# mirage/decompress

Hardware: AMD Instinct MI355X
Metric: MiB/s inflate over N zlib streams (uncompressed bytes / wall second) (higher is better)
Workload: dtype u8; 1 GPU; C2: 4096 x 256 KiB zlib streams per GPU, dynamic Huffman (libz level 6; even streams = slices of the reference's test/corpus, odd = order-2 Markov ASCII text, 64 symbols, seed 0xC2 + i, SURVEY 8(d)), Zl.Inf.Ns semantics, one stream per pair of wavefronts (decoder + copier); streams_per_gpu=4096, stream_bytes=262144, unique_streams=4096

## Files before the change

### decompress_amd/csrc/inflate_wave.hip

```cpp
#ifndef MD_RMAX
#define MD_RMAX 576
#endif
#ifndef MD_STAGE
#define MD_STAGE 5248
#endif
#ifndef MD_PAIR_OCC
#define MD_PAIR_OCC 5
#endif
#include "inflate_wave_core.hpp"

namespace md {
namespace wv {

#ifdef MD_DEBUG_KNOWN_BOUNDS
constexpr uint32_t KB_ROUNDS = 512;
__device__ uint4 *g_kb_buf;
__device__ int g_kb_mode;
#endif
struct Sink {
  lds_u8 *stage;
  uint8_t *g;
  uint32_t cap;
  uint32_t pos;
  uint32_t lane;
  uint32_t a, b;
  bool want_adler;
  __device__ __forceinline__ uint32_t sbase() const { return pos & ~15u; }

  __device__ __forceinline__ void flush(uint32_t total) {
    const uint32_t rb = sbase();
    const uint32_t endp = pos + total;
    const uint32_t full0 = (pos + 15) & ~15u, full1 = endp & ~15u;
    uint32_t s1 = 0, s2 = 0;
    for (uint32_t ps = full0; ps < full1; ps += 1024) {
      const uint32_t cpos = ps + lane * 16;
      if (cpos < full1) {
        const lds_u32 *sp = reinterpret_cast<const lds_u32 *>(stage + (cpos - rb));
        const uint32_t w0 = sp[0], w1 = sp[1], w2 = sp[2], w3 = sp[3];
        const uint4 v = make_uint4(w0, w1, w2, w3);
        __builtin_memcpy(g + cpos, &v, 16);
        if (want_adler) {
          uint32_t t1 = __builtin_amdgcn_udot4(w0, 0x01010101u, 0u, false);
          t1 = __builtin_amdgcn_udot4(w1, 0x01010101u, t1, false);
          t1 = __builtin_amdgcn_udot4(w2, 0x01010101u, t1, false);
          t1 = __builtin_amdgcn_udot4(w3, 0x01010101u, t1, false);
          uint32_t tk = __builtin_amdgcn_udot4(w0, 0x03020100u, 0u, false);
          tk = __builtin_amdgcn_udot4(w1, 0x07060504u, tk, false);
          tk = __builtin_amdgcn_udot4(w2, 0x0b0a0908u, tk, false);
          tk = __builtin_amdgcn_udot4(w3, 0x0f0e0d0cu, tk, false);
          s1 += t1;
          s2 += (endp - cpos) * t1 - tk;
        }
      }
    }
    {
      const uint32_t head1 = full0 < endp ? full0 : endp;
      const uint32_t tail0 = full1 > head1 ? full1 : head1;
      const uint32_t x = lane < 16 ? pos + lane : tail0 + (lane - 16);
      if (lane < 16 ? x < head1 : (lane < 32 && x < endp)) {
        const uint32_t d = stage[x - rb];
        g[x] = (uint8_t)d;
        s1 += d;
        s2 += (endp - x) * d;
      }
    }
    if (want_adler) {
      s1 = wave_sum(s1);
      s2 = wave_sum(s2 % 65521u);
      b = (b + total * a + s2) % 65521u;
      a = (a + s1) % 65521u;
    }
    pos = endp;
  }
};

constexpr int FR = RMAX / kWave;
struct FarRow {
  uint32_t qs, n, src;
  bool near, has;
  uint32_t ml;
};
__device__ __forceinline__ FarRow far_row(const lds_u32 *mrec, const lds_u16 *mpos, uint32_t r, uint32_t nrec, uint32_t rb, uint32_t R0) {
  FarRow f;
  f.has = r < nrec;
  const uint32_t tk = mrec[f.has ? r : 0u];
  f.qs = mpos[f.has ? r : 0u];
  const uint32_t d = (tk & 0x7fff) + 1;
  f.ml = ((tk >> 16) & 0xff) + 3;
  const uint32_t s = rb + f.qs - d;
  f.near = f.has && (tk & kNearBit);
  const uint32_t head = s < R0 ? R0 - s : 0u;
  f.n = !f.has ? 0u : f.near ? head : f.ml;
  f.src = f.n ? s : 0u;
  return f;
}
template <class PF>
__device__ __forceinline__ void copy_far(const lds_u32 *mrec, const lds_u16 *mpos, lds_u16 *list, const Sink &sk,
                                         uint32_t lane, uint32_t nrec, uint32_t *nnear_out, PF &pf) {
  lds_u8 *stage = sk.stage;
  const uint32_t R0 = sk.pos, rb = sk.sbase();
  const uint8_t *g = sk.g;
  uint32_t nnear = 0;
  uint64_t v0[FR], v1[FR];
  uint32_t pk[FR];
  uint32_t nlong = 0;
  bool spill = false;
#pragma unroll
  for (int u = 0; u < FR; u++) {
    const FarRow f = far_row(mrec, mpos, u * kWave + lane, nrec, rb, R0);
    v0[u] = out_ld64(g + f.src);
    v1[u] = out_ld64(g + f.src + 8);
    pk[u] = f.qs | (f.n << 16);
    const uint64_t nb = __ballot(f.near);
    if (f.near) list[nnear + lane_rank(nb)] = (uint16_t)(u * kWave + lane);
    nnear += (uint32_t)__builtin_popcountll(nb);
    const uint64_t lb = __ballot(f.n > 16);
    const uint32_t lc = (uint32_t)__builtin_popcountll(lb);
    if (nnear + nlong + lc > RMAX) {
      spill = true;
      nlong = 0;
    }
    if (lb && !spill) {
      if (f.n > 16) list[RMAX - 1 - (nlong + lane_rank(lb))] = (uint16_t)(u * kWave + lane);
      nlong += lc;
    }
  }
  pf.tick_lds(P_FAR_REC);
#pragma unroll
  for (int u = 0; u < FR; u++) {
    if ((uint32_t)u * kWave < nrec) {
      const uint32_t qs = pk[u] & 0xffffu, n = pk[u] >> 16;
      if constexpr (PF::on) {
        if (u == 0) {
          asm volatile("" ::"v"(v0[u]), "v"(v1[u]));
          pf.tick_all(P_FAR_LOAD);
        }
      }
      if (n) {
        lds_u8 *dd = stage + qs;
        lds_put(dd, v0[u], n < 8 ? n : 8);
        if (n > 8) lds_put(dd + 8, v1[u], n < 16 ? n - 8 : 8);
      }
    }
  }
  pf.tick_lds(P_FAR);
  for (uint32_t c0 = 0; c0 < nlong; c0 += kWave) {
    const bool has = c0 + lane < nlong;
    const uint32_t r = has ? list[RMAX - 1 - (c0 + lane)] : 0u;
    const FarRow f = far_row(mrec, mpos, r, nrec, rb, R0);
    const uint32_t n = has ? f.n : 0u;
    const uint64_t w0 = out_ld64(g + (n ? f.src + 16 : 0u)), w1 = out_ld64(g + (n ? f.src + 24 : 0u));
    if (n) {
      lds_u8 *dd = stage + f.qs + 16;
      lds_put(dd, w0, n < 24 ? n - 16 : 8);
      if (n > 24) lds_put(dd + 8, w1, n < 32 ? n - 24 : 8);
    }
    for (uint64_t lm = __ballot(n > 32); lm;) {
      uint32_t ln[4], lsrc[4], lqs[4];
      uint64_t d[4];
#pragma unroll
      for (int k = 0; k < 4; k++) {
        const bool any = lm != 0;
        const uint32_t l = any ? (uint32_t)__builtin_ctzll(lm) : 0u;
        lm &= lm - 1;
        ln[k] = any ? rdlane(n, l) : 0u;
        lsrc[k] = rdlane(f.src, l);
        lqs[k] = rdlane(f.qs, l);
      }
      const uint32_t j = 32 + lane * 8;
#pragma unroll
      for (int k = 0; k < 4; k++) d[k] = out_ld64(g + (j < ln[k] ? lsrc[k] + j : 0u));
#pragma unroll
      for (int k = 0; k < 4; k++)
        if (j < ln[k]) lds_put(stage + lqs[k] + j, d[k], ln[k] - j < 8 ? ln[k] - j : 8);
    }
  }
  if (spill) {
    pf.count(C_FAR_SPILL);
    for (uint32_t c0 = 0; c0 < nrec; c0 += kWave) {
      const FarRow f = far_row(mrec, mpos, c0 + lane, nrec, rb, R0);
      for (uint64_t lm = __ballot(f.n > 16); lm; lm &= lm - 1) {
        const uint32_t l = (uint32_t)__builtin_ctzll(lm);
        const uint32_t ln = rdlane(f.n, l), lsrc = rdlane(f.src, l), lqs = rdlane(f.qs, l);
        const uint32_t j = 16 + lane * 8;
        if (j < ln) lds_put(stage + lqs + j, out_ld64(g + lsrc + j), ln - j < 8 ? ln - j : 8);
      }
    }
  }
  pf.tick_all(P_FAR);
  *nnear_out = nnear;
}
template <class PF>
__device__ __noinline__ void copy_far_guarded(const lds_u32 *mrec, const lds_u16 *mpos, lds_u16 *list,
                                              lds_u8 *stage, const uint8_t *g, uint32_t R0, uint32_t rb, uint32_t cap,
                                              uint32_t lane, uint32_t nrec, uint32_t *nnear_out) {
  uint32_t nnear = 0;
  for (uint32_t c0 = 0; c0 < nrec; c0 += kWave) {
    const uint32_t r = c0 + lane;
    const bool has = r < nrec;
    const uint32_t tk = mrec[has ? r : 0u], qs = mpos[has ? r : 0u];
    const uint32_t d = (tk & 0x7fff) + 1, ml = ((tk >> 16) & 0xff) + 3;
    const uint32_t s = rb + qs - d;
    const bool near = has && (tk & kNearBit);
    uint32_t n = has ? ml : 0u;
    const uint64_t nb = __ballot(near);
    if (near) {
      list[nnear + lane_rank(nb)] = (uint16_t)r;
      n = s < R0 ? R0 - s : 0u;
    }
    nnear += (uint32_t)__builtin_popcountll(nb);
    for (uint32_t j = 0; j < n; j += 8) lds_put(stage + qs + j, out_ld_guard(g, s + j, n - j, cap), n - j < 8 ? n - j : 8);
  }
  *nnear_out = nnear;
}

__device__ __forceinline__ void wave_copy(lds_u8 *stage, uint32_t dd, uint32_t ss, uint32_t n, uint32_t d, uint32_t lane) {
  if (d >= n) {
    const uint32_t j = lane * 8;
    if (j < n) lds_put(stage + dd + j, lds_ld64(stage + ss + j), n - j < 8 ? n - j : 8);
  } else if (d < 8) {
    uint64_t v = lds_ld64(stage + ss);
    const uint32_t sh = 8 * d;
    v &= (1ull << sh) - 1;
    v |= v << sh;
    if (2 * sh < 64) v |= v << (2 * sh);
    if (4 * sh < 64) v |= v << (4 * sh);
    const uint32_t adv = (0x76586880u >> (4 * d)) & 15;
    const uint32_t j = lane * adv;
    if (j < n) lds_put(stage + dd + j, v, n - j < adv ? n - j : adv);
  } else {
    const float inv = 1.0f / (float)d;
    for (uint32_t j = lane * 4; j < n; j += 4 * kWave) {
      uint32_t r = j - (uint32_t)((float)j * inv) * d;
      r = (int32_t)r < 0 ? r + d : r;
      r = r >= d ? r - d : r;
      uint32_t w = 0;
#pragma unroll
      for (uint32_t k = 0; k < 4; k++) {
        const uint32_t x = r + k >= d ? r + k - d : r + k;
        w |= (uint32_t)stage[ss + x] << (8 * k);
      }
      lds_put(stage + dd + j, w, n - j < 4 ? n - j : 4);
    }
  }
}

template <class PF>
__device__ __forceinline__ void copy_near_all(const lds_u32 *mrec, const lds_u16 *mpos, const lds_u16 *list,
                                              const Sink &sk, uint32_t lane, uint32_t count, bool *stuck, PF &pf) {
  lds_u8 *stage = sk.stage;
  const uint32_t head = sk.pos - sk.sbase();
  for (uint32_t c0 = 0; c0 < count; c0 += kWave) {
    bool todo = c0 + lane < count;
    const uint32_t e = todo ? list[c0 + lane] : 0u;
    const uint32_t tk = mrec[e], qs = mpos[e];
    const uint32_t d = (tk & 0x7fff) + 1, ml = ((tk >> 16) & 0xff) + 3;
    const int32_t s0 = (int32_t)qs - (int32_t)d;
    const uint32_t skip = s0 < (int32_t)head ? head - (uint32_t)s0 : 0u;
    const uint32_t sa = (uint32_t)(s0 + (int32_t)skip), sb = d < ml ? qs : (uint32_t)s0 + ml;
    const uint32_t n = ml - skip;
    const bool fast = d >= n && n <= 32;
    const uint32_t qb = todo ? qs + skip : 0xffffffffu, qe = todo ? qs + ml : 0xffffffffu;
    uint32_t jlo = 0, jhi = 0;
#pragma unroll
    for (uint32_t st = 32; st > 0; st >>= 1) {
      const uint32_t ve = __shfl(qe, jlo + st - 1), vb = __shfl(qb, jhi + st - 1);
      jlo = ve <= sa ? jlo + st : jlo;
      jhi = vb < sb ? jhi + st : jhi;
    }
    jhi = jhi < lane ? jhi : lane;
    uint64_t need = 0;
    if (sa < sb && jlo < jhi) need = ((jhi >= 64 ? 0ull : (1ull << jhi)) - 1ull) & ~((1ull << jlo) - 1ull);
    uint64_t done = 0;
    pf.tick_lds(P_NEAR_LOAD);
    for (uint32_t guard = 0; __ballot(todo) != 0; guard++) {
      if (guard > kWave) {
        *stuck = true;
        return;
      }
      pf.count(C_NEAR_IT);
      const bool ready = todo && (need & ~done) == 0;
      if constexpr (PF::on) {
        if (__ballot(ready && !fast)) pf.count(C_LONG_NEAR);
      }
      pf.tick_lds(P_NEAR);
      if (ready && fast) {
        lds_u8 *dd = stage + qs + skip;
        const lds_u8 *ss = stage + sa;
        const uint64_t v0 = lds_ld64(ss), v1 = lds_ld64(ss + 8), v2 = lds_ld64(ss + 16), v3 = lds_ld64(ss + 24);
        lds_put(dd, v0, n < 8 ? n : 8);
        if (n > 8) lds_put(dd + 8, v1, n < 16 ? n - 8 : 8);
        if (n > 16) {
          lds_put(dd + 16, v2, n < 24 ? n - 16 : 8);
          if (n > 24) lds_put(dd + 24, v3, n - 24);
        }
      }
      pf.tick_lds(P_NEAR_FAST);
      for (uint64_t lm = __ballot(ready && !fast); lm; lm &= lm - 1) {
        const uint32_t l = (uint32_t)__builtin_ctzll(lm);
        wave_copy(stage, rdlane(qs + skip, l), rdlane(sa, l), rdlane(n, l), rdlane(d, l), lane);
      }
      pf.tick_lds(P_NEAR_SLOW);
      done |= __ballot(ready);
      todo = todo && !ready;
      pf.tick_lds(P_NEAR_UPD);
    }
  }
  pf.tick(P_NEAR);
}

template <class PF>
__device__ __forceinline__ void copy_round(lds_smem *sm, Sink &sk, uint32_t lane, uint32_t total, uint32_t nrec, bool *stuck, PF &pf) {
  const lds_u32 *mrec = (const lds_u32 *)sm->mrec;
  const lds_u16 *mpos = (const lds_u16 *)sm->mpos;
  lds_u16 *list = (lds_u16 *)sm->list;
  const uint32_t R0 = sk.pos, rb = sk.sbase();
  uint32_t nnear = 0;
#ifdef MD_DEBUG_KNOWN_BOUNDS
  {
    const int kbm = __builtin_amdgcn_readfirstlane(g_kb_mode);
    if (kbm & 8) {
      sk.pos += total;
      return;
    }
    if (kbm & 4) {
      sk.flush(total);
      return;
    }
  }
#endif
  __builtin_amdgcn_fence(__ATOMIC_RELEASE, "workgroup");
  if (R0 + 40 > sk.cap) {
    copy_far_guarded<PF>(mrec, mpos, list, sk.stage, sk.g, R0, rb, sk.cap, lane, nrec, &nnear);
    pf.tick(P_FAR);
  } else {
    copy_far(mrec, mpos, list, sk, lane, nrec, &nnear, pf);
  }
  copy_near_all(mrec, mpos, list, sk, lane, nnear, stuck, pf);
  sk.flush(total);
  pf.tick(P_ADLER);
}

__device__ __forceinline__ uint32_t mail_ld(const MD_LDS uint32_t *p) {
  return __hip_atomic_load(p, __ATOMIC_RELAXED, __HIP_MEMORY_SCOPE_WORKGROUP);
}
__device__ __forceinline__ void mail_st(MD_LDS uint32_t *p, uint32_t v) {
  __hip_atomic_store(p, v, __ATOMIC_RELAXED, __HIP_MEMORY_SCOPE_WORKGROUP);
}
__device__ __forceinline__ bool mail_wait_idle(lds_smem *sm, uint32_t sent) {
  while (uni(mail_ld(&sm->mail.copied)) != sent) __builtin_amdgcn_s_sleep(2);
  asm volatile("" ::: "memory");
  return uni(mail_ld(&sm->mail.stuck)) == 0;
}
__device__ __forceinline__ void mail_post(lds_smem *sm, uint32_t lane, uint32_t kind, uint32_t total, uint32_t x, uint32_t &sent) {
  if (lane == 0) {
    sm->mail.kind = kind;
    sm->mail.total = total;
    sm->mail.x = x;
  }
  asm volatile("s_waitcnt lgkmcnt(0)" ::: "memory");
  sent++;
  if (lane == 0) mail_st(&sm->mail.emitted, sent);
}

template <class PF, bool PAIR, bool BUDGET>
__device__ __forceinline__ int inflate_block(lds_smem *sm, const uint8_t *__restrict__ body, uint32_t body_len, Sink &sk,
                                             uint32_t lroot, uint32_t lane, uint32_t *bp_io, uint32_t *zone_io, Window &wnd,
                                             uint32_t &sent, PF &pf) {
  uint32_t bp = *bp_io;
  lds_u32 *win = (lds_u32 *)sm->win;
  const lds_u32 *lut = (const lds_u32 *)sm->lut;
  lds_u32 *mrec = (lds_u32 *)sm->mrec;
  lds_u16 *mpos = (lds_u16 *)sm->mpos;
  const uint32_t total_bits = body_len * 8;
  uint32_t zs = *zone_io;
  constexpr bool kSplit = PAIR && !BUDGET && MD_EMIT_SPLIT != 0;
  for (;;) {
    const uint32_t base = (bp >> 5) << 2;
    wnd.ensure(win, body, body_len, base, lane);
    const uint32_t rbp = bp - base * 8, tot = total_bits - base * 8;
    pf.tick(P_ENSURE);
    pf.count(C_ROUNDS);
    pf.count(C_PASSES);
    uint32_t start = rbp + lane * zs, end = 0, stop = 0, nb = 0;
    uint32_t midp = 0xffffffffu, midcnt = 0;
    const uint32_t limit = rbp + (lane + 1) * zs;
    const uint32_t runin_ = (zs * RUNIN_NUM) / RUNIN_DEN, runin = runin_ < lane * zs ? runin_ : lane * zs;
    bool counted = false;
#ifdef MD_DEBUG_KNOWN_BOUNDS
    const int kbm = __builtin_amdgcn_readfirstlane(g_kb_mode);
    const bool kb_can = wnd.kb_round < KB_ROUNDS;
    uint4 *kbp = g_kb_buf + ((size_t)wnd.kb_sid * KB_ROUNDS + wnd.kb_round) * kWave + lane;
    wnd.kb_round++;
    if ((kbm & 3) == 2 && kb_can) {
      const uint4 v = *kbp;
      start = v.x;
      end = v.y;
      stop = v.z & 0xffffu;
      counted = (v.z >> 16) != 0;
      nb = v.w;
    } else {
#endif
    sync_pass<false, BUDGET>(win, lut, lroot, true, start - runin, limit, end, stop, nb);
    pf.tick(P_DECODE1);
    const uint32_t passes = zs * PASSES >= PASS_BITS ? PASSES : PASS_BITS / zs > PASSES_MAX ? PASSES_MAX : PASS_BITS / zs;
    for (uint32_t it = 0; it < passes; it++) {
      const uint32_t pe = wave_shr1(end), ps = wave_shr1(stop);
      const bool redo = lane == 0 ? !counted : (ps == 0 && (pe != start || !counted));
      if (__ballot(redo) == 0) break;
      if (redo && lane > 0) start = pe;
      pf.count(C_PASSES);
      if constexpr (kSplit) sync_pass<true, BUDGET, true>(win, lut, lroot, redo, start, limit, end, stop, nb, limit - (zs * MD_SPLIT_B) / 8, &midp, &midcnt);
      else sync_pass<true, BUDGET>(win, lut, lroot, redo, start, limit, end, stop, nb);
      counted = counted || redo;
    }
#ifdef MD_DEBUG_KNOWN_BOUNDS
      if ((kbm & 3) == 1 && kb_can) *kbp = make_uint4(start, end, stop | (counted ? 0x10000u : 0u), nb);
    }
#endif
    pf.tick(P_DECODE2);
    uint32_t nvalid;
    {
      const uint32_t pe = wave_shr1(end), ps = wave_shr1(stop);
      const uint64_t bad = __ballot(!counted || (lane > 0 && (ps != 0 || pe != start)));
      nvalid = bad ? (uint32_t)__builtin_ctzll(bad) : 64;
    }
    const uint32_t R0 = sk.pos, rb = sk.sbase();
    uint32_t mynb = lane < nvalid ? nb : 0;
    const uint32_t off = wave_excl_scan(mynb, lane);
    if (nvalid < 64) pf.count(C_END_CHAIN);
    {
      const uint32_t bend = ((off + mynb) & (kCountMatch - 1)), rend = (off + mynb) >> 20;
      const uint64_t fits = __ballot((R0 - rb) + bend <= STAGE - 16 && rend <= RMAX);
      const uint32_t nfit = fits == ~0ull ? 64 : (uint32_t)__builtin_ctzll(~fits);
      if (nfit < nvalid) {
        pf.count(rdlane(rend, nfit) > RMAX ? C_END_RECORDS : C_END_FIT);
        nvalid = nfit ? nfit : 1;
      }
    }
    const bool mine = lane < nvalid;
    if (!mine) mynb = 0;
    const uint32_t boff = off & (kCountMatch - 1), roff = off >> 20;
    const uint32_t q0 = R0 + boff;
    LaneOut lo;
    lo.endp = end;
    lo.stopc = 0;
    lo.bytes = 0;
    lo.nm = 0;
    if constexpr (PAIR) {
      pf.tick(P_DECODE2);
      if (!mail_wait_idle(sm, sent)) return MD_E_HIP;
      pf.tick(P_WAIT_DEC);
    }
    bool split = false;
    uint32_t bq = 0, br = 0;
    LaneOut lob;
    lob.endp = 0, lob.stopc = 0, lob.bytes = 0, lob.nm = 0;
    bool gob = false;
    if constexpr (kSplit) split = zs >= 128;
    {
      const uint32_t all = rdlane(off + mynb, nvalid - 1) & (kCountMatch - 1);
      const bool plain = tot >= rbp + kWave * zs + 64 && R0 >= 32768u && all <= sk.cap - R0 && (R0 - rb) + all <= STAGE - 16;
      uint32_t alimit = limit;
      if constexpr (kSplit) {
        if (split) {
          gob = mine && midp != 0xffffffffu && midp < limit && midp >= start;
          bq = midcnt & (kCountMatch - 1);
          br = midcnt >> 20;
          lds_u32 *hx = reinterpret_cast<lds_u32 *>(sm->list);
          hx[4 * lane + 0] = gob ? midp : 0xffffffffu;
          hx[4 * lane + 1] = limit;
          hx[4 * lane + 2] = q0 + bq;
          hx[4 * lane + 3] = roff + br;
          if (lane < 6) hx[kHxUni + lane] = lane == 0 ? lroot : lane == 1 ? tot : lane == 2 ? rb : lane == 3 ? R0 : lane == 4 ? sk.cap : (plain ? 0u : 1u);
          mail_post(sm, lane, kJobEmit, 0, 0, sent);
          alimit = gob ? midp : limit;
        }
      }
      if (plain && !BUDGET) emit_pass<false, false>(win, lut, lroot, mrec, mpos, sk.stage, roff, tot, mine, start, alimit, q0, rb, R0, sk.cap, lo);
      else emit_pass<true, BUDGET>(win, lut, lroot, mrec, mpos, sk.stage, roff, tot, mine, start, alimit, q0, rb, R0, sk.cap, lo);
      if constexpr (kSplit) {
        if (split) {
          if (!mail_wait_idle(sm, sent)) return MD_E_HIP;
          const lds_u32 *hx = reinterpret_cast<const lds_u32 *>(sm->list);
          if (gob) {
            lob.endp = hx[4 * lane + 0];
            lob.stopc = hx[4 * lane + 1];
            lob.bytes = hx[4 * lane + 2];
            lob.nm = hx[4 * lane + 3];
          }
          const bool sa = lo.stopc != 0;
          if (!sa && gob) {
            lo.endp = lob.endp;
            lo.stopc = lob.stopc;
            lo.bytes = bq + lob.bytes;
            lo.nm = br + lob.nm;
          }
        }
      }
    }
    pf.tick(P_EMIT_A);
    uint32_t total, lstop, nrec;
    {
      const uint64_t fm = __ballot(mine && lo.stopc != 0);
      if (fm) {
        const uint32_t fl = __builtin_ctzll(fm);
        lstop = rdlane(lo.stopc, fl);
        total = rdlane(boff, fl) + rdlane(lo.bytes, fl);
        nrec = rdlane(roff, fl) + rdlane(lo.nm, fl);
        if (lstop == kStEob) pf.count(C_END_EOB);
        else if (lstop == kStTrunc) pf.count(C_END_STAGE);
        nvalid = fl + 1;
      } else {
        lstop = 0;
        const uint32_t all = rdlane(off + mynb, nvalid - 1);
        total = all & (kCountMatch - 1);
        nrec = all >> 20;
      }
    }
    const uint32_t nbp = base * 8 + rdlane(lo.endp, nvalid - 1);
    wnd.fetch(body, body_len, (nbp >> 5) << 2, lane);
    bool stuck = false;
    if constexpr (PAIR) {
      mail_post(sm, lane, kJobRound, total, nrec, sent);
      sk.pos += total;
    } else {
      copy_round(sm, sk, lane, total, nrec, &stuck, pf);
    }
    pf.count(C_LANES, nvalid);
    if (stuck || (nbp == bp && total == 0 && (lstop == 0 || lstop == kStTrunc))) return MD_E_HIP;
    {
      const uint32_t bits = nbp - bp;
      const uint64_t want = (uint64_t)(STAGE - STAGE / 8) * bits / ((uint64_t)kWave * (total ? total : 1u));
      zs = want > S ? S : want < SMIN ? SMIN : (uint32_t)want;
    }
    bp = nbp;
    if (lstop == kStEob) break;
    if (lstop != 0 && lstop != kStTrunc) return (int)lstop;
  }
  *bp_io = bp;
  *zone_io = zs;
  return MD_OK;
}

__device__ __forceinline__ void copy_stored(Sink &sk, const uint8_t *__restrict__ body, uint32_t p, uint32_t len, uint32_t lane) {
  const uint8_t *q = body + p;
  uint32_t left = len;
  while (left) {
    const uint32_t seg = left < STAGE - 16 ? left : STAGE - 16;
    const uint32_t s0 = sk.pos - sk.sbase();
    for (uint32_t j = lane; j < seg; j += kWave) sk.stage[s0 + j] = q[j];
    sk.flush(seg);
    q += seg;
    left -= seg;
  }
}

template <class PF>
__device__ __forceinline__ void copier_main(lds_smem *sm, const uint8_t *__restrict__ body, Sink &sk, uint32_t lane, PF &pf) {
  uint32_t done = 0;
  for (;;) {
    while (uni(mail_ld(&sm->mail.emitted)) == done) __builtin_amdgcn_s_sleep(2);
    asm volatile("" ::: "memory");
    const uint32_t kind = uni(sm->mail.kind), total = uni(sm->mail.total), x = uni(sm->mail.x);
    pf.tick(P_WAIT_COPY);
    if (kind == kJobQuit) break;
    bool stuck = false;
    if (kind == kJobRound) copy_round(sm, sk, lane, total, x, &stuck, pf);
    else if (kind == kJobEmit) {
      if constexpr (MD_EMIT_SPLIT != 0) {
        lds_u32 *hx = reinterpret_cast<lds_u32 *>(sm->list);
        const uint32_t bstart = hx[4 * lane + 0], blimit = hx[4 * lane + 1], bq0 = hx[4 * lane + 2], brec = hx[4 * lane + 3];
        const uint32_t lroot = uni(hx[kHxUni + 0]), tot = uni(hx[kHxUni + 1]), rb = uni(hx[kHxUni + 2]), R0 = uni(hx[kHxUni + 3]),
                       cap = uni(hx[kHxUni + 4]), checked = uni(hx[kHxUni + 5]);
        const bool go = bstart != 0xffffffffu;
        LaneOut lo;
        lo.endp = bstart, lo.stopc = 0, lo.bytes = 0, lo.nm = 0;
        const lds_u32 *win = (const lds_u32 *)sm->win;
        const lds_u32 *lut = (const lds_u32 *)sm->lut;
        if (checked) emit_pass<true, false>(win, lut, lroot, (lds_u32 *)sm->mrec, (lds_u16 *)sm->mpos, sk.stage, brec, tot, go, go ? bstart : 0u, blimit, bq0, rb, R0, cap, lo);
        else emit_pass<false, false>(win, lut, lroot, (lds_u32 *)sm->mrec, (lds_u16 *)sm->mpos, sk.stage, brec, tot, go, go ? bstart : 0u, blimit, bq0, rb, R0, cap, lo);
        hx[4 * lane + 0] = lo.endp;
        hx[4 * lane + 1] = lo.stopc;
        hx[4 * lane + 2] = lo.bytes;
        hx[4 * lane + 3] = lo.nm;
      }
    } else copy_stored(sk, body, x, total, lane);
    if (lane == 0) {
      sm->mail.a = sk.a;
      sm->mail.b = sk.b;
      if (stuck) sm->mail.stuck = 1;
    }
    asm volatile("s_waitcnt lgkmcnt(0)" ::: "memory");
    done++;
    if (lane == 0) mail_st(&sm->mail.copied, done);
  }
}

template <bool PROF, bool PAIR>
__global__ __launch_bounds__(PAIR ? 2 * kWave : kWave, PAIR ? MD_PAIR_OCC : 2) void inflate_wave_kernel(
    int format, uint32_t n, const uint8_t *__restrict__ in, const uint64_t *__restrict__ in_off,
    const uint64_t *__restrict__ in_len, uint8_t *out, const uint64_t *__restrict__ out_off,
    const uint64_t *__restrict__ out_cap, uint64_t *__restrict__ out_len,
    uint64_t *__restrict__ consumed, int32_t *__restrict__ status, uint32_t *__restrict__ checksum,
    uint64_t *__restrict__ dbg, const uint32_t *__restrict__ order, Cont cont) {
  __shared__ Smem smem;
  lds_smem *sm = (lds_smem *)&smem;
  Prof<PROF> pf;
  pf.init();
  const uint32_t lane = threadIdx.x & (kWave - 1);
  const uint32_t wave = PAIR ? uni(threadIdx.x / kWave) : 0u;
  if (blockIdx.x >= n) return;
  const uint32_t sid = order ? order[blockIdx.x] : blockIdx.x;

  const uint8_t *src = in + in_off[sid];
  uint64_t slen64 = in_len[sid], cap64 = out_cap[sid];
  if (slen64 > MD_MAX_INFLATE_IN) {
    if (threadIdx.x == 0) {
      out_len[sid] = 0;
      consumed[sid] = 0;
      status[sid] = MD_E_INVALID_ARGUMENT;
      if (checksum) checksum[sid] = 0;
    }
    return;
  }
  const uint32_t slen = (uint32_t)slen64;
  const bool cap_clamped = cap64 > MD_MAX_STREAM;
  const uint32_t cap = cap_clamped ? (uint32_t)MD_MAX_STREAM : (uint32_t)cap64;

  int rc = MD_OK;
  uint32_t body_off = 0, body_len = slen;
  if (format == MD_FORMAT_ZLIB) {
    if (slen < 2) rc = MD_UNEXPECTED_END_OF_INPUT;
    else {
      uint32_t cmf = src[0], flg = src[1];
      if (((cmf << 8) + flg) % 31 != 0 || (cmf & 0xf) != 8) rc = MD_INVALID_HEADER;
      else if (slen < 6) rc = MD_UNEXPECTED_END_OF_INPUT;
      else {
        body_off = 2;
        body_len = slen - 6;
      }
    }
  }
  const uint8_t *body = src + body_off;

  Sink sk;
  sk.stage = (lds_u8 *)sm->stage;
  sk.g = out + out_off[sid];
  sk.cap = cap;
  const uint32_t hist = cont.hist_len ? cont.hist_len[sid] : 0u, adler0 = cont.adler_in ? cont.adler_in[sid] : 1u;
  sk.pos = hist < cap ? hist : cap;
  sk.lane = lane;
  sk.a = adler0 & 0xffffu;
  sk.b = adler0 >> 16;
  sk.want_adler = (checksum != nullptr) || format == MD_FORMAT_ZLIB || cont.resume_adler != nullptr;

  if (threadIdx.x < 4) sm->lut[kStopEobI + threadIdx.x] = mk_entry(0, 0, 0, 0, kStopEobI + (threadIdx.x & 2));
  if constexpr (PAIR) {
    if (threadIdx.x < sizeof(Mail) / 4) ((lds_u32 *)&sm->mail)[threadIdx.x] = threadIdx.x == 6 ? sk.a : threadIdx.x == 7 ? sk.b : 0u;
    __syncthreads();
    if (wave == 1) {
      copier_main(sm, body, sk, lane, pf);
      if constexpr (PROF) {
        if (lane == 0 && sid == 0 && dbg) {
          const int mine[] = {P_FAR, P_NEAR, P_ADLER, P_NEAR_FAST, P_NEAR_SLOW, P_NEAR_UPD, P_NEAR_LOAD, P_FAR_REC, P_FAR_LOAD, P_WAIT_COPY};
          for (int i : mine) dbg[i] = pf.acc[i];
          dbg[P_COUNT + C_NEAR_IT] = pf.cnt[C_NEAR_IT];
          dbg[P_COUNT + C_LONG_NEAR] = pf.cnt[C_LONG_NEAR];
          dbg[P_COUNT + C_FAR_SPILL] = pf.cnt[C_FAR_SPILL];
        }
      }
      return;
    }
  }

  lds_u32 *win = (lds_u32 *)sm->win;
  const uint32_t total_bits = body_len * 8;
  uint32_t bp = cont.start_bit ? cont.start_bit[sid] & 7u : 0u;
  uint32_t zone = S;
  uint32_t sent = 0;
  uint32_t fixed_lroot = 0;
  Window wnd;
  wnd.base = 0xffffffffu;
#ifdef MD_DEBUG_KNOWN_BOUNDS
  wnd.kb_round = 0;
  wnd.kb_sid = sid;
#endif
  if (cont.resume_bits && lane == 0) {
    cont.resume_bits[sid] = bp;
    cont.resume_out[sid] = sk.pos;
    cont.resume_adler[sid] = adler0;
    cont.resume_last[sid] = 0;
  }

  if (rc == MD_OK) {
    bool last = false;
    uint32_t lds_base = 0xffffffffu;
    while (!last && rc == MD_OK) {
      uint32_t base = (bp >> 5) << 2;
      if (lds_base != 0xffffffffu && bp >= lds_base * 8 && bp - lds_base * 8 <= 4096) base = lds_base;
      else {
        wnd.ensure(win, body, body_len, base, lane);
        lds_base = base;
      }
      uint32_t rbp = bp - base * 8;
      const uint32_t tot = total_bits - base * 8;
      if ((int32_t)(tot - rbp) < 3) {
        rc = MD_UNEXPECTED_END_OF_INPUT;
        break;
      }
      const uint32_t hdr = uni(peek(win, rbp));
      last = hdr & 1;
      uint32_t type = (hdr >> 1) & 3;
      bp += 3;
      rbp += 3;
      bool block_done = false;
      if (type == 1) {
        for (;;) {
          if (rbp + 7 > tot || rbp + 64 > WIN_WORDS * 32 - 64 || (uni(peek(win, rbp)) & 0x7fu) != 0) break;
          rbp += 7;
          bp += 7;
          block_done = true;
          if (last || rbp + 3 > tot) break;
          const uint32_t h = uni(peek(win, rbp)) & 7u;
          if (((h >> 1) & 3) != 1) break;
          last = h & 1;
          rbp += 3;
          bp += 3;
          block_done = false;
        }
      }
      if (block_done) {
      } else if (type == 0) {
        uint32_t p = (bp + 7) >> 3;
        if (body_len - p < 4) {
          rc = MD_UNEXPECTED_END_OF_INPUT;
          break;
        }
// ... 197 lines not shown
```

### decompress_amd/csrc/inflate_wave_core.hpp

```cpp
#pragma once
#include <stdlib.h>
#include "inflate_util.hpp"
#include "internal.hpp"

#if !defined(MD_RMAX) || !defined(MD_STAGE)
#error "define MD_RMAX and MD_STAGE before inflate_wave_core.hpp"
#endif

namespace md {
namespace wv {

constexpr uint32_t S = 264;
constexpr uint32_t SMIN = 48;
constexpr uint32_t KMAX = 64;
#ifndef MD_EMIT_SPLIT
#define MD_EMIT_SPLIT 1
#endif
#if defined(MD_DEBUG_KNOWN_BOUNDS)
#undef MD_EMIT_SPLIT
#define MD_EMIT_SPLIT 0
#endif
#ifndef MD_SPLIT_B
#define MD_SPLIT_B 4
#endif
#ifndef MD_RUNIN_NUM
#define MD_RUNIN_NUM 3
#define MD_RUNIN_DEN 2
#endif
constexpr uint32_t RUNIN_NUM = MD_RUNIN_NUM, RUNIN_DEN = MD_RUNIN_DEN;
constexpr uint32_t PASSES = 5;
constexpr uint32_t PASS_BITS = 1600, PASSES_MAX = 16;
constexpr uint32_t RMAX = MD_RMAX;
constexpr uint32_t STAGE = MD_STAGE;
constexpr uint32_t WIN_WORDS = 544;

constexpr uint32_t kLitSize = 852, kDistSize = 592;
constexpr uint32_t kLitRootMax = 512;
constexpr uint32_t kLitSubB = 0;
constexpr uint32_t kDistB = kLitSize - kLitRootMax;
constexpr uint32_t kLitB = kDistB + kDistSize;
constexpr uint32_t kStopEobI = kLitB + kLitRootMax;
constexpr uint32_t kStopBadI = kStopEobI + 2;
constexpr uint32_t kLutWords = kStopBadI + 2;
constexpr uint32_t kTbMask = 0xffe00000u;
constexpr uint32_t kLoopy = 0x100u;
static_assert(kDistB % 2 == 0 && kLitB % 2 == 0 && kStopEobI % 2 == 0 && kLutWords == 1448, "even table bases");
constexpr uint32_t kStEob = 100, kStTrunc = 101;
constexpr uint32_t kCountMatch = 1u << 20;
constexpr uint32_t kNearBit = 0x8000u;

struct Mail {
  uint32_t emitted;
  uint32_t copied;
  uint32_t kind;
  uint32_t total;
  uint32_t x;
  uint32_t stuck;
  uint32_t a, b;
};
constexpr uint32_t kJobRound = 0, kJobStored = 1, kJobQuit = 2, kJobEmit = 3;
constexpr uint32_t kHxUni = 4 * 64;
struct Smem {
  uint32_t win[WIN_WORDS];
  uint32_t lut[kLutWords];
  uint32_t mrec[RMAX];
  uint16_t mpos[RMAX];
  alignas(16) uint8_t stage[STAGE + 16];
  uint16_t list[RMAX];
  Mail mail;
};
struct HScratch {
  uint8_t lens[384];
  uint16_t work[320];
  uint32_t ctr;
};
#if MD_RMAX == 576 && MD_STAGE == 5248
static_assert(sizeof(Smem) <= 17920, "9 streams (18 wavefronts) per CU: 160 KiB / 9, in whole 512-byte units");
#endif
static_assert(RMAX % 64 == 0 && STAGE % 16 == 0 && RMAX * 2 >= (kHxUni + 6) * 4, "record rows, staging chunks, the emit job's words in `list`");
constexpr uint32_t kHScratchAt = 1136;
static_assert(kHScratchAt >= 4 + 572 + 8 && kHScratchAt % 16 == 0 && kHScratchAt + sizeof(HScratch) <= WIN_WORDS * 4, "header scratch lives behind the header's bits");
typedef MD_LDS Smem lds_smem;
typedef MD_LDS HScratch lds_hscratch;
__device__ __forceinline__ lds_hscratch *hscratch_of(lds_smem *sm) {
  return reinterpret_cast<lds_hscratch *>(reinterpret_cast<lds_u8 *>(sm->win) + kHScratchAt);
}

__device__ __forceinline__ uint32_t mk_entry(uint32_t n, uint32_t xb, uint32_t val8, uint32_t nbits, uint32_t tb) {
  return n | (xb << 5) | (val8 << 9) | (nbits << 17) | (tb << 21);
}
__device__ __forceinline__ uint32_t e_n(uint32_t e) { return e & 31; }
__device__ __forceinline__ uint32_t e_xb(uint32_t e) { return (e >> 5) & 15; }
__device__ __forceinline__ uint32_t e_val(uint32_t e) { return (e >> 9) & 255; }
__device__ __forceinline__ uint32_t e_tb(uint32_t e) { return e >> 21; }
__device__ __forceinline__ bool e_link(uint32_t e) { return e_tb(e) < kLitB && e_tb(e) != kDistB; }
__device__ __forceinline__ uint32_t e_root(uint32_t lroot) { return mk_entry(0, 0, 0, lroot, kLitB); }
__device__ __forceinline__ uint32_t lit_leaf(uint32_t sym, uint32_t codelen, uint32_t lroot, uint32_t droot) {
  if (sym < 256) return mk_entry(codelen, 0, sym, lroot, kLitB);
  if (sym == 256) return mk_entry(codelen, 0, 0, 0, kStopEobI);
  const uint32_t l = (sym - 257) & 31;
  const uint32_t xb = (l >= 8 && l < 28) ? (l - 4) >> 2 : 0;
  const uint32_t base3 = l < 8 ? l : l < 28 ? (4 + (l & 3)) << xb : l == 28 ? 255 : 0;
  return mk_entry(codelen + xb, xb, base3, droot, kDistB);
}
__device__ __forceinline__ uint32_t dist_leaf(uint32_t dv, uint32_t codelen, uint32_t lroot) {
  dv &= 31;
  if (dv >= 30) return mk_entry(codelen, 0, 0, 0, kStopBadI);
  const uint32_t xb = dv >= 4 ? (dv - 2) >> 1 : 0;
  const uint32_t m = dv < 4 ? dv : ((dv & 1) | 2);
  return mk_entry(codelen + xb, xb, m, lroot, kLitB);
}
__device__ __forceinline__ uint32_t dist_value(uint32_t m, uint32_t xb, uint32_t x) { return (m << xb) + 1 + x; }

struct Window {
  uint32_t w[8], wx;
  uint32_t base;
#ifdef MD_DEBUG_KNOWN_BOUNDS
  uint32_t kb_round, kb_sid;
#endif
  __device__ __forceinline__ void fetch(const uint8_t *__restrict__ body, uint32_t nbytes, uint32_t b, uint32_t lane) {
    base = b;
    const uint32_t off = b + lane * 32;
#pragma unroll
    for (int k = 0; k < 8; k++) w[k] = 0;
    if (off + 32 <= nbytes) __builtin_memcpy(w, body + off, 32);
    else if (off < nbytes)
      for (uint32_t k = 0; k < 32 && off + k < nbytes; k++) w[k >> 2] |= (uint32_t)body[off + k] << (8 * (k & 3));
    wx = 0;
    if (lane < WIN_WORDS - 512) {
      const uint32_t ox = b + 2048 + lane * 4;
      if (ox + 4 <= nbytes) __builtin_memcpy(&wx, body + ox, 4);
      else if (ox < nbytes)
        for (uint32_t k = 0; k < 4 && ox + k < nbytes; k++) wx |= (uint32_t)body[ox + k] << (8 * k);
    }
  }
  __device__ __forceinline__ void put(lds_u32 *win, uint32_t lane) const {
    lds_u32 *dst = win + lane * 8;
#pragma unroll
    for (int k = 0; k < 8; k++) dst[k] = w[k];
    if (lane < WIN_WORDS - 512) win[512 + lane] = wx;
  }
  __device__ __forceinline__ void ensure(lds_u32 *win, const uint8_t *__restrict__ body, uint32_t nbytes, uint32_t b, uint32_t lane) {
    if (base != b) fetch(body, nbytes, b, lane);
    put(win, lane);
    base = 0xffffffffu;
  }
};
__device__ __forceinline__ uint32_t peek(const lds_u32 *win, uint32_t p) {
  const lds_u32 *q = reinterpret_cast<const lds_u32 *>(reinterpret_cast<const lds_u8 *>(win) + ((p >> 3) & ~3u));
  return __builtin_amdgcn_alignbit(q[1], q[0], p & 31);
}
__device__ __forceinline__ uint32_t lut_at(const lds_u32 *lut, uint32_t tb, uint32_t idx) {
  return *reinterpret_cast<const lds_u32 *>(reinterpret_cast<const lds_u8 *>(lut) + ((tb + idx) << 2));
}

struct UBits {
  const lds_u32 *win;
  uint64_t buf;
  uint32_t n;
  uint32_t wp;
  __device__ __forceinline__ void init(const lds_u32 *w, uint32_t bp) {
    win = w;
    wp = bp >> 5;
    buf = ((uint64_t)uni(win[wp]) | ((uint64_t)uni(win[wp + 1]) << 32)) >> (bp & 31);
    n = 64 - (bp & 31);
    wp += 2;
  }
  __device__ __forceinline__ uint32_t pos() const { return wp * 32 - n; }
  __device__ __forceinline__ void fill() {
    if (n <= 32) {
      buf |= (uint64_t)uni(win[wp]) << n;
      n += 32;
      wp++;
    }
  }
  __device__ __forceinline__ uint32_t peekb(uint32_t k) const { return (uint32_t)buf & ((1u << k) - 1); }
  __device__ __forceinline__ void drop(uint32_t k) {
    buf >>= k;
    n -= k;
  }
};

struct Canon {
  uint32_t cnt[16];
  uint32_t first[16];
  uint32_t offs[16];
  uint32_t max, min, root, left;
};
__device__ __forceinline__ uint32_t lane_rank(uint64_t m) {
  return __builtin_amdgcn_mbcnt_hi((uint32_t)(m >> 32), __builtin_amdgcn_mbcnt_lo((uint32_t)m, 0));
}
template <int K>
__device__ __forceinline__ void canon_counts(const uint32_t (&len)[K], uint32_t rootpref, Canon &c) {
#pragma unroll
  for (int l = 1; l < 16; l++) {
    uint32_t n = 0;
#pragma unroll
    for (int k = 0; k < K; k++) n += (uint32_t)__builtin_popcountll(__ballot(len[k] == (uint32_t)l));
    c.cnt[l] = n;
  }
  c.cnt[0] = 0;
  c.max = 0;
  c.min = 16;
#pragma unroll
  for (int l = 15; l >= 1; l--) {
    if (c.cnt[l] && c.max == 0) c.max = l;
    if (c.cnt[l]) c.min = l;
  }
  int left = 1;
  bool over = false;
  uint32_t code = 0, off = 0;
  c.first[0] = 0;
  c.offs[0] = 0;
#pragma unroll
  for (int l = 1; l < 16; l++) {
    left = (left << 1) - (int)c.cnt[l];
    over = over || left < 0;
    code = (code + c.cnt[l - 1]) << 1;
    c.first[l] = code;
    c.offs[l] = off;
    off += c.cnt[l];
  }
  c.left = over ? 0xffffffffu : (uint32_t)left;
  uint32_t root = rootpref;
  if (root > c.max) root = c.max;
  if (root < c.min) root = c.min;
  c.root = root;
}

template <int K, class LEAF>
__device__ __forceinline__ bool build_walk(const uint32_t (&len)[K], const Canon &c, lds_u32 *lut, uint32_t tb0, uint32_t sub0,
                                           uint32_t size, lds_hscratch *hs, uint32_t lane, uint32_t zero_entry, LEAF leaf) {
// ... 412 lines not shown
```

Measured before the change: 248,900 MiB/s.

## Add compaction-based near-copy sweep, pack emit handoff words, batch far rows

Adds an optional near-match path (MD_NEAR_LIST=0) that rebuilds near-record groups from per-row ballot masks via ds_permute compaction instead of keeping a near list in LDS. This lets the list array shrink to a fixed size. The emit job's per-lane handoff is packed from four words into two, and copy_far processes rows in batches of at most nine to cap register arrays. The slice-size heuristic now also limits rounds by record capacity, and new static asserts allow alternative RMAX/STAGE configs for higher occupancy. The default build still uses the near-list path, so most of the structural change only takes effect when the macros are changed.

```diff
diff --git a/decompress_amd/csrc/inflate_wave.hip b/decompress_amd/csrc/inflate_wave.hip
--- a/decompress_amd/csrc/inflate_wave.hip
+++ b/decompress_amd/csrc/inflate_wave.hip
@@ -75,6 +75,7 @@
 };
 
 constexpr int FR = RMAX / kWave;
+constexpr int FRB = FR < 9 ? FR : 9;
 struct FarRow {
   uint32_t qs, n, src;
   bool near, has;
@@ -96,39 +97,46 @@
 }
 template <class PF>
 __device__ __forceinline__ void copy_far(const lds_u32 *mrec, const lds_u16 *mpos, lds_u16 *list, const Sink &sk,
-                                         uint32_t lane, uint32_t nrec, uint32_t *nnear_out, PF &pf) {
+                                         uint32_t lane, uint32_t nrec, uint32_t *nnear_out, uint32_t *nlo_out, uint32_t *nhi_out, PF &pf) {
   lds_u8 *stage = sk.stage;
   const uint32_t R0 = sk.pos, rb = sk.sbase();
   const uint8_t *g = sk.g;
-  uint32_t nnear = 0;
-  uint64_t v0[FR], v1[FR];
-  uint32_t pk[FR];
+  uint32_t nnear = 0, nlo = 0, nhi = 0;
+  uint64_t v0[FRB], v1[FRB];
+  uint32_t pk[FRB];
   uint32_t nlong = 0;
   bool spill = false;
+  uint32_t b0 = 0;
+  do {
 #pragma unroll
-  for (int u = 0; u < FR; u++) {
-    const FarRow f = far_row(mrec, mpos, u * kWave + lane, nrec, rb, R0);
+  for (int u = 0; u < FRB; u++) {
+    const FarRow f = far_row(mrec, mpos, b0 + u * kWave + lane, nrec, rb, R0);
     v0[u] = out_ld64(g + f.src);
     v1[u] = out_ld64(g + f.src + 8);
     pk[u] = f.qs | (f.n << 16);
     const uint64_t nb = __ballot(f.near);
-    if (f.near) list[nnear + lane_rank(nb)] = (uint16_t)(u * kWave + lane);
-    nnear += (uint32_t)__builtin_popcountll(nb);
+    if constexpr (kNearList) {
+      if (f.near) list[nnear + lane_rank(nb)] = (uint16_t)(b0 + u * kWave + lane);
+      nnear += (uint32_t)__builtin_popcountll(nb);
+    } else if (lane == b0 / kWave + u) {
+      nlo = (uint32_t)nb;
+      nhi = (uint32_t)(nb >> 32);
+    }
     const uint64_t lb = __ballot(f.n > 16);
     const uint32_t lc = (uint32_t)__builtin_popcountll(lb);
-    if (nnear + nlong + lc > RMAX) {
+    if (nlong + lc > kLongCap || nnear + nlong + lc > kListN) {
       spill = true;
       nlong = 0;
     }
     if (lb && !spill) {
-      if (f.n > 16) list[RMAX - 1 - (nlong + lane_rank(lb))] = (uint16_t)(u * kWave + lane);
+      if (f.n > 16) list[kListN - 1 - (nlong + lane_rank(lb))] = (uint16_t)(b0 + u * kWave + lane);
       nlong += lc;
     }
   }
   pf.tick_lds(P_FAR_REC);
 #pragma unroll
-  for (int u = 0; u < FR; u++) {
-    if ((uint32_t)u * kWave < nrec) {
+  for (int u = 0; u < FRB; u++) {
+    if (b0 + (uint32_t)u * kWave < nrec) {
       const uint32_t qs = pk[u] & 0xffffu, n = pk[u] >> 16;
       if constexpr (PF::on) {
         if (u == 0) {
@@ -143,10 +151,12 @@
       }
     }
   }
+  b0 += FRB * kWave;
+  } while (FR > FRB && b0 < nrec);
   pf.tick_lds(P_FAR);
   for (uint32_t c0 = 0; c0 < nlong; c0 += kWave) {
     const bool has = c0 + lane < nlong;
-    const uint32_t r = has ? list[RMAX - 1 - (c0 + lane)] : 0u;
+    const uint32_t r = has ? list[kListN - 1 - (c0 + lane)] : 0u;
     const FarRow f = far_row(mrec, mpos, r, nrec, rb, R0);
     const uint32_t n = has ? f.n : 0u;
     const uint64_t w0 = out_ld64(g + (n ? f.src + 16 : 0u)), w1 = out_ld64(g + (n ? f.src + 24 : 0u));
@@ -189,6 +199,8 @@
   }
   pf.tick_all(P_FAR);
   *nnear_out = nnear;
+  *nlo_out = nlo;
+  *nhi_out = nhi;
 }
 template <class PF>
 __device__ __noinline__ void copy_far_guarded(const lds_u32 *mrec, const lds_u16 *mpos, lds_u16 *list,
@@ -203,12 +215,12 @@
     const uint32_t s = rb + qs - d;
     const bool near = has && (tk & kNearBit);
     uint32_t n = has ? ml : 0u;
-    const uint64_t nb = __ballot(near);
-    if (near) {
-      list[nnear + lane_rank(nb)] = (uint16_t)r;
-      n = s < R0 ? R0 - s : 0u;
-    }
-    nnear += (uint32_t)__builtin_popcountll(nb);
+    if (near) n = s < R0 ? R0 - s : 0u;
+    if constexpr (kNearList) {
+      const uint64_t nb = __ballot(near);
+      if (near) list[nnear + lane_rank(nb)] = (uint16_t)r;
+      nnear += (uint32_t)__builtin_popcountll(nb);
+    }
     for (uint32_t j = 0; j < n; j += 8) lds_put(stage + qs + j, out_ld_guard(g, s + j, n - j, cap), n - j < 8 ? n - j : 8);
   }
   *nnear_out = nnear;
@@ -246,65 +258,114 @@
 }
 
 template <class PF>
-__device__ __forceinline__ void copy_near_all(const lds_u32 *mrec, const lds_u16 *mpos, const lds_u16 *list,
-                                              const Sink &sk, uint32_t lane, uint32_t count, bool *stuck, PF &pf) {
-  lds_u8 *stage = sk.stage;
+__device__ __forceinline__ bool copy_near_group(const lds_u32 *mrec, const lds_u16 *mpos, lds_u8 *stage, uint32_t head,
+                                                uint32_t lane, uint32_t e, uint32_t count, PF &pf) {
+  bool todo = lane < count;
+  e = todo ? e : 0u;
+  const uint32_t tk = mrec[e], qs = mpos[e];
+  const uint32_t d = (tk & 0x7fff) + 1, ml = ((tk >> 16) & 0xff) + 3;
+  const int32_t s0 = (int32_t)qs - (int32_t)d;
+  const uint32_t skip = s0 < (int32_t)head ? head - (uint32_t)s0 : 0u;
+  const uint32_t sa = (uint32_t)(s0 + (int32_t)skip), sb = d < ml ? qs : (uint32_t)s0 + ml;
+  const uint32_t n = ml - skip;
+  const bool fast = d >= n && n <= 32;
+  const uint32_t qb = todo ? qs + skip : 0xffffffffu, qe = todo ? qs + ml : 0xffffffffu;
+  uint32_t jlo = 0, jhi = 0;
+#pragma unroll
+  for (uint32_t st = 32; st > 0; st >>= 1) {
+    const uint32_t ve = __shfl(qe, jlo + st - 1), vb = __shfl(qb, jhi + st - 1);
+    jlo = ve <= sa ? jlo + st : jlo;
+    jhi = vb < sb ? jhi + st : jhi;
+  }
+  jhi = jhi < lane ? jhi : lane;
+  uint64_t need = 0;
+  if (sa < sb && jlo < jhi) need = ((jhi >= 64 ? 0ull : (1ull << jhi)) - 1ull) & ~((1ull << jlo) - 1ull);
+  uint64_t done = 0;
+  pf.tick_lds(P_NEAR_LOAD);
+  for (uint32_t guard = 0; __ballot(todo) != 0; guard++) {
+    if (guard > kWave) return false;
+    pf.count(C_NEAR_IT);
+    const bool ready = todo && (need & ~done) == 0;
+    if constexpr (PF::on) {
+      if (__ballot(ready && !fast)) pf.count(C_LONG_NEAR);
+    }
+    pf.tick_lds(P_NEAR);
+    if (ready && fast) {
+      lds_u8 *dd = stage + qs + skip;
+      const lds_u8 *ss = stage + sa;
+      const uint64_t v0 = lds_ld64(ss), v1 = lds_ld64(ss + 8), v2 = lds_ld64(ss + 16), v3 = lds_ld64(ss + 24);
+      lds_put(dd, v0, n < 8 ? n : 8);
+      if (n > 8) lds_put(dd + 8, v1, n < 16 ? n - 8 : 8);
+      if (n > 16) {
+        lds_put(dd + 16, v2, n < 24 ? n - 16 : 8);
+        if (n > 24) lds_put(dd + 24, v3, n - 24);
+      }
+    }
+    pf.tick_lds(P_NEAR_FAST);
+    for (uint64_t lm = __ballot(ready && !fast); lm; lm &= lm - 1) {
+      const uint32_t l = (uint32_t)__builtin_ctzll(lm);
+      wave_copy(stage, rdlane(qs + skip, l), rdlane(sa, l), rdlane(n, l), rdlane(d, l), lane);
+    }
+    pf.tick_lds(P_NEAR_SLOW);
+    done |= __ballot(ready);
+    todo = todo && !ready;
+    pf.tick_lds(P_NEAR_UPD);
+  }
+  return true;
+}
+template <class PF>
+__device__ __forceinline__ void copy_near_list(const lds_u32 *mrec, const lds_u16 *mpos, const lds_u16 *list, const Sink &sk,
+                                               uint32_t lane, uint32_t count, bool *stuck, PF &pf) {
   const uint32_t head = sk.pos - sk.sbase();
   for (uint32_t c0 = 0; c0 < count; c0 += kWave) {
-    bool todo = c0 + lane < count;
-    const uint32_t e = todo ? list[c0 + lane] : 0u;
-    const uint32_t tk = mrec[e], qs = mpos[e];
-    const uint32_t d = (tk & 0x7fff) + 1, ml = ((tk >> 16) & 0xff) + 3;
-    const int32_t s0 = (int32_t)qs - (int32_t)d;
-    const uint32_t skip = s0 < (int32_t)head ? head - (uint32_t)s0 : 0u;
-    const uint32_t sa = (uint32_t)(s0 + (int32_t)skip), sb = d < ml ? qs : (uint32_t)s0 + ml;
-    const uint32_t n = ml - skip;
-    const bool fast = d >= n && n <= 32;
-    const uint32_t qb = todo ? qs + skip : 0xffffffffu, qe = todo ? qs + ml : 0xffffffffu;
-    uint32_t jlo = 0, jhi = 0;
-#pragma unroll
-    for (uint32_t st = 32; st > 0; st >>= 1) {
-      const uint32_t ve = __shfl(qe, jlo + st - 1), vb = __shfl(qb, jhi + st - 1);
-      jlo = ve <= sa ? jlo + st : jlo;
-      jhi = vb < sb ? jhi + st : jhi;
-    }
-    jhi = jhi < lane ? jhi : lane;
-    uint64_t need = 0;
-    if (sa < sb && jlo < jhi) need = ((jhi >= 64 ? 0ull : (1ull << jhi)) - 1ull) & ~((1ull << jlo) - 1ull);
-    uint64_t done = 0;
-    pf.tick_lds(P_NEAR_LOAD);
-    for (uint32_t guard = 0; __ballot(todo) != 0; guard++) {
-      if (guard > kWave) {
-        *stuck = true;
-        return;
-      }
-      pf.count(C_NEAR_IT);
-      const bool ready = todo && (need & ~done) == 0;
-      if constexpr (PF::on) {
-        if (__ballot(ready && !fast)) pf.count(C_LONG_NEAR);
-      }
-      pf.tick_lds(P_NEAR);
-      if (ready && fast) {
-        lds_u8 *dd = stage + qs + skip;
-        const lds_u8 *ss = stage + sa;
-        const uint64_t v0 = lds_ld64(ss), v1 = lds_ld64(ss + 8), v2 = lds_ld64(ss + 16), v3 = lds_ld64(ss + 24);
-        lds_put(dd, v0, n < 8 ? n : 8);
-        if (n > 8) lds_put(dd + 8, v1, n < 16 ? n - 8 : 8);
-        if (n > 16) {
-          lds_put(dd + 16, v2, n < 24 ? n - 16 : 8);
-          if (n > 24) lds_put(dd + 24, v3, n - 24);
-        }
-      }
-      pf.tick_lds(P_NEAR_FAST);
-      for (uint64_t lm = __ballot(ready && !fast); lm; lm &= lm - 1) {
-        const uint32_t l = (uint32_t)__builtin_ctzll(lm);
-        wave_copy(stage, rdlane(qs + skip, l), rdlane(sa, l), rdlane(n, l), rdlane(d, l), lane);
-      }
-      pf.tick_lds(P_NEAR_SLOW);
-      done |= __ballot(ready);
-      todo = todo && !ready;
-      pf.tick_lds(P_NEAR_UPD);
-    }
+    const uint32_t e = c0 + lane < count ? list[c0 + lane] : 0u;
+    if (!copy_near_group(mrec, mpos, sk.stage, head, lane, e, count - c0 < kWave ? count - c0 : (uint32_t)kWave, pf)) {
+      *stuck = true;
+      return;
+    }
+  }
+  pf.tick(P_NEAR);
+}
+template <class PF, bool REG>
+__device__ __forceinline__ void copy_near_sweep(const lds_u32 *mrec, const lds_u16 *mpos, const Sink &sk, uint32_t lane,
+                                                uint32_t nrec, uint32_t nlo, uint32_t nhi, bool *stuck, PF &pf) {
+  const uint32_t head = sk.pos - sk.sbase();
+  uint32_t grp = 0;
+  uint32_t fill = 0;
+  for (uint32_t c0 = 0;; c0 += kWave) {
+    const bool last = c0 >= nrec;
+    uint32_t cnt = 0, recv = 0;
+    bool got = false;
+    if (!last) {
+      uint64_t nb;
+      if constexpr (REG) {
+        nb = (uint64_t)rdlane(nlo, c0 / kWave) | ((uint64_t)rdlane(nhi, c0 / kWave) << 32);
+      } else {
+        const uint32_t r = c0 + lane;
+        nb = __ballot(r < nrec && (mrec[r < nrec ? r : 0u] & kNearBit));
+      }
+      if (nb == 0) continue;
+      cnt = (uint32_t)__builtin_popcountll(nb);
+      const uint32_t rank = lane_rank(nb);
+      const uint32_t to = (nb >> lane) & 1 ? fill + rank : fill + cnt + (lane - rank);
+      recv = (uint32_t)__builtin_amdgcn_ds_permute((int)((to & (kWave - 1)) << 2), (int)(c0 + lane));
+      got = ((lane - fill) & (kWave - 1)) < cnt;
+      if (fill + cnt < kWave) {
+        if (got) grp = recv;
+        fill += cnt;
+        continue;
+      }
+      if (got && lane >= fill) grp = recv;
+    } else if (fill == 0) {
+      break;
+    }
+    if (!copy_near_group(mrec, mpos, sk.stage, head, lane, grp, last ? fill : (uint32_t)kWave, pf)) {
+      *stuck = true;
+      return;
+    }
+    if (last) break;
+    if (got && lane < fill) grp = recv;
+    fill = fill + cnt - kWave;
   }
   pf.tick(P_NEAR);
 }
@@ -333,10 +394,13 @@
   if (R0 + 40 > sk.cap) {
     copy_far_guarded<PF>(mrec, mpos, list, sk.stage, sk.g, R0, rb, sk.cap, lane, nrec, &nnear);
     pf.tick(P_FAR);
+    if constexpr (!kNearList) copy_near_sweep<PF, false>(mrec, mpos, sk, lane, nrec, 0, 0, stuck, pf);
   } else {
-    copy_far(mrec, mpos, list, sk, lane, nrec, &nnear, pf);
-  }
-  copy_near_all(mrec, mpos, list, sk, lane, nnear, stuck, pf);
+    uint32_t nlo, nhi;
+    copy_far(mrec, mpos, list, sk, lane, nrec, &nnear, &nlo, &nhi, pf);
+    if constexpr (!kNearList) copy_near_sweep<PF, true>(mrec, mpos, sk, lane, nrec, nlo, nhi, stuck, pf);
+  }
+  if constexpr (kNearList) copy_near_list(mrec, mpos, list, sk, lane, nnear, stuck, pf);
   sk.flush(total);
   pf.tick(P_ADLER);
 }
@@ -468,10 +532,8 @@
           bq = midcnt & (kCountMatch - 1);
           br = midcnt >> 20;
           lds_u32 *hx = reinterpret_cast<lds_u32 *>(sm->list);
-          hx[4 * lane + 0] = gob ? midp : 0xffffffffu;
-          hx[4 * lane + 1] = limit;
-          hx[4 * lane + 2] = q0 + bq;
-          hx[4 * lane + 3] = roff + br;
+          hx[2 * lane + 0] = (gob ? midp : kHxIdle) | ((limit & 0x7fffu) << 16);
+          hx[2 * lane + 1] = ((q0 + bq - rb) & 0xffffu) | ((roff + br) << 16);
           if (lane < 6) hx[kHxUni + lane] = lane == 0 ? lroot : lane == 1 ? tot : lane == 2 ? rb : lane == 3 ? R0 : lane == 4 ? sk.cap : (plain ? 0u : 1u);
           mail_post(sm, lane, kJobEmit, 0, 0, sent);
           alimit = gob ? midp : limit;
@@ -484,10 +546,11 @@
           if (!mail_wait_idle(sm, sent)) return MD_E_HIP;
           const lds_u32 *hx = reinterpret_cast<const lds_u32 *>(sm->list);
           if (gob) {
-            lob.endp = hx[4 * lane + 0];
-            lob.stopc = hx[4 * lane + 1];
-            lob.bytes = hx[4 * lane + 2];
-            lob.nm = hx[4 * lane + 3];
+            const uint32_t w0 = hx[2 * lane + 0], w1 = hx[2 * lane + 1];
+            lob.endp = w0 & 0xffffu;
+            lob.stopc = w0 >> 16;
+            lob.bytes = w1 & 0xffffu;
+            lob.nm = w1 >> 16;
           }
           const bool sa = lo.stopc != 0;
           if (!sa && gob) {
@@ -531,7 +594,11 @@
     if (stuck || (nbp == bp && total == 0 && (lstop == 0 || lstop == kStTrunc))) return MD_E_HIP;
     {
       const uint32_t bits = nbp - bp;
-      const uint64_t want = (uint64_t)(STAGE - STAGE / 8) * bits / ((uint64_t)kWave * (total ? total : 1u));
+      uint64_t want = (uint64_t)(STAGE - STAGE / 8) * bits / ((uint64_t)kWave * (total ? total : 1u));
+      if (nrec) {
+        const uint64_t wr = (uint64_t)RMAX * bits / ((uint64_t)kWave * nrec);
+        want = wr < want ? wr : want;
+      }
       zs = want > S ? S : want < SMIN ? SMIN : (uint32_t)want;
     }
     bp = nbp;
@@ -570,20 +637,19 @@
     else if (kind == kJobEmit) {
       if constexpr (MD_EMIT_SPLIT != 0) {
         lds_u32 *hx = reinterpret_cast<lds_u32 *>(sm->list);
-        const uint32_t bstart = hx[4 * lane + 0], blimit = hx[4 * lane + 1], bq0 = hx[4 * lane + 2], brec = hx[4 * lane + 3];
+        const uint32_t w0 = hx[2 * lane + 0], w1 = hx[2 * lane + 1];
         const uint32_t lroot = uni(hx[kHxUni + 0]), tot = uni(hx[kHxUni + 1]), rb = uni(hx[kHxUni + 2]), R0 = uni(hx[kHxUni + 3]),
                        cap = uni(hx[kHxUni + 4]), checked = uni(hx[kHxUni + 5]);
-        const bool go = bstart != 0xffffffffu;
+        const uint32_t bstart = w0 & 0x7fffu, blimit = w0 >> 16, bq0 = rb + (w1 & 0xffffu), brec = w1 >> 16;
+        const bool go = bstart != kHxIdle;
         LaneOut lo;
         lo.endp = bstart, lo.stopc = 0, lo.bytes = 0, lo.nm = 0;
         const lds_u32 *win = (const lds_u32 *)sm->win;
         const lds_u32 *lut = (const lds_u32 *)sm->lut;
         if (checked) emit_pass<true, false>(win, lut, lroot, (lds_u32 *)sm->mrec, (lds_u16 *)sm->mpos, sk.stage, brec, tot, go, go ? bstart : 0u, blimit, bq0, rb, R0, cap, lo);
         else emit_pass<false, false>(win, lut, lroot, (lds_u32 *)sm->mrec, (lds_u16 *)sm->mpos, sk.stage, brec, tot, go, go ? bstart : 0u, blimit, bq0, rb, R0, cap, lo);
-        hx[4 * lane + 0] = lo.endp;
-        hx[4 * lane + 1] = lo.stopc;
-        hx[4 * lane + 2] = lo.bytes;
-        hx[4 * lane + 3] = lo.nm;
+        hx[2 * lane + 0] = lo.endp | (lo.stopc << 16);
+        hx[2 * lane + 1] = lo.bytes | (lo.nm << 16);
       }
     } else copy_stored(sk, body, x, total, lane);
     if (lane == 0) {
diff --git a/decompress_amd/csrc/inflate_wave_core.hpp b/decompress_amd/csrc/inflate_wave_core.hpp
--- a/decompress_amd/csrc/inflate_wave_core.hpp
+++ b/decompress_amd/csrc/inflate_wave_core.hpp
@@ -59,14 +59,21 @@
   uint32_t a, b;
 };
 constexpr uint32_t kJobRound = 0, kJobStored = 1, kJobQuit = 2, kJobEmit = 3;
-constexpr uint32_t kHxUni = 4 * 64;
+constexpr uint32_t kHxUni = 2 * 64;
+constexpr uint32_t kHxIdle = 0x7fffu;
+#ifndef MD_NEAR_LIST
+#define MD_NEAR_LIST 1
+#endif
+constexpr bool kNearList = MD_NEAR_LIST != 0;
+constexpr uint32_t kHxWords = 272, kLongCap = 96;
+constexpr uint32_t kListN = kNearList && RMAX > kHxWords ? RMAX : kHxWords;
 struct Smem {
   uint32_t win[WIN_WORDS];
   uint32_t lut[kLutWords];
   uint32_t mrec[RMAX];
   uint16_t mpos[RMAX];
   alignas(16) uint8_t stage[STAGE + 16];
-  uint16_t list[RMAX];
+  uint16_t list[kListN];
   Mail mail;
 };
 struct HScratch {
@@ -74,10 +81,15 @@
   uint16_t work[320];
   uint32_t ctr;
 };
-#if MD_RMAX == 576 && MD_STAGE == 5248
+#if (MD_RMAX == 576 && MD_STAGE == 5248) || (MD_RMAX == 640 && MD_STAGE == 5520)
 static_assert(sizeof(Smem) <= 17920, "9 streams (18 wavefronts) per CU: 160 KiB / 9, in whole 512-byte units");
 #endif
-static_assert(RMAX % 64 == 0 && STAGE % 16 == 0 && RMAX * 2 >= (kHxUni + 6) * 4, "record rows, staging chunks, the emit job's words in `list`");
+#if MD_RMAX == 576 && MD_STAGE == 4368
+static_assert(sizeof(Smem) <= 16384, "10 streams (20 wavefronts) per CU: 160 KiB / 10");
+#endif
+static_assert(RMAX % 64 == 0 && STAGE % 16 == 0 && kHxWords * 2 >= (kHxUni + 6) * 4 && kLongCap <= kHxWords,
+              "record rows, staging chunks, the emit job's words and the long records in `list`");
+static_assert(STAGE <= 8192 && RMAX < 1024 && (WIN_WORDS + 2) * 32 < 0x7fff, "the emit job's packed words: 13-bit positions, 10-bit records, 15-bit window bits");
 constexpr uint32_t kHScratchAt = 1136;
 static_assert(kHScratchAt >= 4 + 572 + 8 && kHScratchAt % 16 == 0 && kHScratchAt + sizeof(HScratch) <= WIN_WORDS * 4, "header scratch lives behind the header's bits");
 typedef MD_LDS Smem lds_smem;
```

Measured after the change: 250,500 MiB/s (median of 6 runs). No clear change (+0.6%).
